# hiroharu-kato/neural_renderer

Hardware: AMD Instinct MI355X
Metric: rasterize fwd+bwd Mpixels/sec @256x256 batch=64 (higher is better)
Workload: dtype f32

## Files before the change

### include/nr_hip.h

```cpp
#ifndef NR_HIP_H
#define NR_HIP_H

#include <stddef.h>
#include <stdint.h>

#ifdef __cplusplus
extern "C" {
#endif

#define NR_VERSION 600

#define NR_E_NULL (-1)
#define NR_E_SIZE (-2)
#define NR_E_WORKSPACE (-3)
#define NR_E_MODE (-4)
#define NR_E_INDEX (-6)

#define NR_FLAG_FIX_TEXTURE_BATCH_Z 1
#define NR_FLAG_EXACT_GRADIENT 2
#define NR_FLAG_K6_GLOBAL 4
#define NR_FLAG_K6_SCAN 8

#define NR_FLAG_ZBUF_EPOCH 16
#define NR_ZBUF_EPOCH_FLAGS(e) (NR_FLAG_ZBUF_EPOCH | (((e) & 0xff) << 8))
#define NR_FLAG_SPARSE_WEIGHT_MAP 32
#define NR_FLAG_SERIAL_BACKWARD 64

#define NR_FLAG_K6_LEGACY 128
#define NR_FLAG_K6_PX 65536
#define NR_FLAG_SHARED_TEXTURES 131072


int nr_version(void);
const char *nr_error_string(int code);

size_t nr_forward_workspace_bytes(int32_t batch_size, int32_t num_faces, int32_t image_size);

size_t nr_backward_workspace_bytes(int32_t batch_size, int32_t num_faces, int32_t image_size,
                                   int32_t return_rgb, int32_t return_alpha);

int nr_forward_face_index_map(const float *faces, int32_t *face_index_map, float *weight_map, float *depth_map,
                              float *face_inv_map, uint8_t *visible_faces, int32_t batch_size, int32_t num_faces,
                              int32_t image_size, double near, double far, void *workspace, size_t workspace_bytes,
                              void *stream);

int nr_forward_texture_sampling(const float *faces, const float *faces_z_ref, const float *textures,
                                const int32_t *face_index_map, const float *weight_map, const float *depth_map,
                                float *rgb_map, int32_t *sampling_index_map, float *sampling_weight_map,
                                const float *background, int32_t bg_per_batch, float *alpha_map, int32_t batch_size,
                                int32_t num_faces, int32_t image_size, int32_t texture_size, double eps, int32_t flags,
                                void *stream);

int nr_backward_pixel_map(const float *faces, const int32_t *face_index_map, const float *rgb_map,
                          const float *alpha_map, const float *grad_rgb_map, const float *grad_alpha_map,
                          float *grad_faces, int32_t batch_size, int32_t num_faces, int32_t image_size, double eps,
                          int32_t return_rgb, int32_t return_alpha, int32_t flags, const uint8_t *visible_faces,
                          void *workspace, size_t workspace_bytes, void *stream);

int nr_backward_textures(const int32_t *face_index_map, const float *sampling_weight_map,
                         const int32_t *sampling_index_map, const float *faces, const float *faces_z_ref,
                         const float *weight_map, const float *depth_map, const float *grad_rgb_map, float *grad_textures,
                         int32_t batch_size, int32_t num_faces, int32_t image_size, int32_t texture_size, double eps,
// ... 473 lines not shown
```

### neural_renderer_amd/_lib.py

```python
import ctypes
import os

import torch

from . import _build

_CONTIGUOUS = torch.contiguous_format

_c = ctypes
_vp, _i32, _f64, _sz = _c.c_void_p, _c.c_int32, _c.c_double, _c.c_size_t


class Camera(_c.Structure):
    _fields_ = [('mode', _i32), ('perspective', _i32), ('target', _c.c_float * 3), ('up', _c.c_float * 3),
                ('width', _c.c_float)]


class Light(_c.Structure):
    _fields_ = [('intensity_ambient', _c.c_float), ('intensity_directional', _c.c_float),
                ('color_ambient', _c.c_float * 3), ('color_directional', _c.c_float * 3), ('direction', _c.c_float * 3)]


class FaceLight(_c.Structure):
    _fields_ = [('light', _vp), ('texture_faces', _i32), ('textures', _vp), ('grad_light', _vp)]
# ... 12 lines not shown
    _fields_ = [('images', _vp), ('image_table', _vp), ('faces_uv', _vp), ('face_image', _vp), ('base', _vp),
                ('texture_size', _i32), ('num_images', _i32), ('num_pixels', _i32), ('image_batch', _i32)]


class Lights(_c.Structure):
    _fields_ = [('intensity_ambient', _vp), ('intensity_directional', _vp), ('color_ambient', _vp),
                ('color_directional', _vp), ('direction', _vp), ('sh', _vp), ('per_image', _i32)]


class LightsGrad(_c.Structure):
    _fields_ = [('intensity_ambient', _vp), ('intensity_directional', _vp), ('color_ambient', _vp),
                ('color_directional', _vp), ('direction', _vp), ('sh', _vp)]


_cam_p, _light_p, _fl_p, _proj_p = _c.POINTER(Camera), _c.POINTER(Light), _c.POINTER(FaceLight), _c.POINTER(Projection)
_uv_p, _cl_p = _c.POINTER(UVImagesStruct), _c.POINTER(CornerLight)
_lights_p, _lights_grad_p = _c.POINTER(Lights), _c.POINTER(LightsGrad)

SIGNATURES = {
    'nr_version': (_c.c_int, []),
    'nr_error_string': (_c.c_char_p, [_c.c_int]),
    'nr_forward_workspace_bytes': (_sz, [_i32, _i32, _i32]),
    'nr_backward_workspace_bytes': (_sz, [_i32, _i32, _i32, _i32, _i32]),
    'nr_forward_face_index_map': (_c.c_int, [_vp] * 6 + [_i32, _i32, _i32, _f64, _f64, _vp, _sz, _vp]),
    'nr_forward_texture_sampling': (_c.c_int, [_vp] * 10 + [_i32, _vp, _i32, _i32, _i32, _i32, _f64, _i32, _vp]),
    'nr_backward_pixel_map': (_c.c_int, [_vp] * 7 + [_i32, _i32, _i32, _f64, _i32, _i32, _i32, _vp, _vp, _sz, _vp]),
    'nr_backward_textures': (_c.c_int, [_vp] * 9 + [_i32, _i32, _i32, _i32, _f64, _i32, _vp]),
    'nr_backward_depth_map': (_c.c_int, [_vp, _vp, _vp, _vp, _vp, _vp, _vp, _i32, _i32, _i32, _vp]),
    'nr_forward_rasterize': (_c.c_int, [_vp] * 10 + [_i32] * 5 + [_f64] * 3 + [_i32, _vp, _sz, _vp]),
    'nr_vertices_to_faces': (_c.c_int, [_vp, _vp, _vp, _i32, _i32, _i32, _i32, _vp]),
    'nr_vertices_to_faces_backward': (_c.c_int, [_vp, _vp, _vp, _i32, _i32, _i32, _i32, _vp]),
    'nr_backward_rasterize': (_c.c_int, [_vp] * 12 + [_i32] * 4 + [_f64, _i32, _vp, _vp, _sz, _vp]),
    'nr_image_epilogue': (_c.c_int, [_vp] * 6 + [_i32] * 3 + [_vp]),
    'nr_image_epilogue_backward': (_c.c_int, [_vp] * 6 + [_i32] * 3 + [_vp]),
    'nr_load_textures': (_c.c_int, [_vp] * 4 + [_i32] * 4 + [_vp]),
    'nr_create_texture_image': (_c.c_int, [_vp] * 3 + [_i32] * 5 + [_vp]),
    'nr_bake_uv_textures': (_c.c_int, [_vp] * 6 + [_i32] * 5 + [_vp]),
    'nr_uv_texture_map_workspace_bytes': (_sz, [_i32] * 4),
    'nr_uv_texture_map': (_c.c_int, [_vp] * 6 + [_i32] * 4 + [_vp, _sz, _vp]),
    'nr_bake_uv_textures_backward': (_c.c_int, [_vp] * 5 + [_i32] * 4 + [_vp]),
    'nr_forward_rasterize_uv': (_c.c_int, [_fl_p, _uv_p] + [_vp] * 8 + [_i32] * 4 + [_f64] * 3 + [_i32, _vp, _sz, _vp]),
    'nr_backward_uv_images_workspace_bytes': (_sz, [_i32] * 4),
    'nr_backward_uv_images': (_c.c_int, [_fl_p, _uv_p] + [_vp] * 6 + [_i32] * 3 + [_f64, _vp, _sz, _vp]),
    'nr_forward_rasterize_uv_smooth': (_c.c_int, [_cl_p, _uv_p] + [_vp] * 8 + [_i32] * 4 + [_f64] * 3 + [_i32, _vp, _sz, _vp]),
    'nr_backward_uv_images_smooth_workspace_bytes': (_sz, [_i32] * 4),
    'nr_backward_uv_images_smooth': (_c.c_int, [_cl_p, _uv_p] + [_vp] * 6 + [_i32] * 3 + [_f64, _vp, _sz, _vp]),
# ... 209 lines not shown
```

### neural_renderer_amd/csrc/nr_backward.hip

```cpp
#include "nr_device.h"
#include "nr_band_lines.h"
#include "nr_k6_tune.h"

using namespace nr;

int nr::plan_backward(const BackwardCall &c, BackwardPlan &p)
{
    p = {};
    const bool fused = c.stages == STAGE_ALL;
    const bool k6 = (c.stages & STAGE_K6) && (c.rgb || c.alpha);
    const bool k7 = (c.stages & STAGE_K7) && (!fused || (c.grad_rgb_map && c.grad_textures));
    const bool k8 = (c.stages & STAGE_K8) && (!fused || c.grad_depth_map);
    const bool sampled = c.sampling_weight_map != nullptr;
    if (!c.faces || !c.face_index_map) return NR_E_NULL;
    if ((c.stages & (STAGE_K6 | STAGE_K8)) && !c.grad_faces) return NR_E_NULL;
    if (c.stages == STAGE_K6 && !k6) return NR_E_MODE;
    if (k6 && c.rgb && (!c.rgb_map || !c.grad_rgb_map)) return NR_E_NULL;
    if (k6 && c.alpha && (!c.alpha_map || !c.grad_alpha_map)) return NR_E_NULL;
    if (k7) {
        if (!c.grad_rgb_map || !c.grad_textures) return NR_E_NULL;
        if ((c.sampling_index_map != nullptr) != sampled) return NR_E_MODE;
        if (!sampled && (!c.weight_map || !c.depth_map)) return NR_E_NULL;
    }
    if (k8 && (!c.depth_map || !c.weight_map || !c.grad_depth_map)) return NR_E_NULL;
    if (int e = check_sizes(c.B, c.F, c.S)) return e;
    if (k6 && (size_t)c.B * c.S * c.S > 0x7fffffffull / 3) return NR_E_SIZE;
    if (k7 && (c.ts < 2 || c.ts > 1024)) return NR_E_SIZE;
    if (k7 && c.lit.light && sampled) return NR_E_MODE;
    if (k7 && (c.flags & NR_FLAG_SHARED_TEXTURES)) return NR_E_MODE;

    const int B = c.B, F = c.F, ts = c.ts;
    p.k6 = k6;
    if (k6) {
        p.k6p = plan_k6(B, F, c.S, c.rgb, c.eps, c.flags);
        p.bands = p.k6p.kernel != K6_KERNEL_GLOBAL;
        if (p.bands && (!c.workspace || c.workspace_bytes < nr_backward_workspace_bytes(B, F, c.S, 1, 0))) return NR_E_WORKSPACE;
    }
    const bool fold = p.bands && k7 && ts <= 13;
    p.gather_first = fold && (size_t)B * F <= k6::SHARED_LAUNCH_MAX_FACES && !(c.flags & NR_FLAG_SERIAL_BACKWARD);
    const bool ts2_static = ts == 2 && (float)(1.0 - c.eps) < 1.0f;
    p.gather_in_tail = k6::TAIL_GATHER_MAX_FACES > 0 && fold && !p.gather_first && !(c.flags & NR_FLAG_SERIAL_BACKWARD) &&
                       ts2_static && !sampled && !c.lit.light && p.k6p.kernel == K6_KERNEL_ROW && !(c.flags & NR_FLAG_EXACT_GRADIENT) &&
                       !p.k6p.row_chunked && c.S <= 512 && (size_t)B * F <= k6::TAIL_GATHER_MAX_FACES;
    const bool gather_early = p.gather_first || p.gather_in_tail;
    p.face_zeros = gather_early ? FACE_ZEROS_ALL : (fold ? FACE_ZEROS_UNLISTED : FACE_ZEROS_NONE);
    p.finish = !p.bands ? FINISH_NONE : gather_early ? (ts <= 8 ? FINISH_BIG : FINISH_ADD) : (fold ? FINISH_GATHER : FINISH_KERNEL);

    if (k7) {
        const size_t n_tex = (size_t)ts * ts * ts * 3;
        p.static_taps = ts2_static && !sampled;
        p.gather = ts <= 13 ? GATHER_FACE : GATHER_ATOMIC;
        p.listed = p.bands && ts <= 13;
        p.lanes = p.static_taps ? 16 : (ts <= 5 ? 16 : (ts <= 8 ? 64 : 256));
        p.gather_lds = p.static_taps ? 0 : (size_t)(256 / p.lanes) * n_tex * sizeof(double);
        p.big = ts <= 8;
        p.depth_in_gather = k8 && ts <= 8 && !sampled && !(ts == 2 && !ts2_static);
        p.tex_bytes = (size_t)B * (c.lit.light ? c.lit.tex_faces : F) * n_tex * sizeof(float);
        if (p.gather_first) {
            p.setup_in_gather = p.k6p.use_records && k6_line_setup_args(c, p.k6p).lds_bytes <= 32768 && p.gather_lds <= 40960;
            if (p.setup_in_gather && !c.lit.light && ((size_t)c.grad_textures & 15) == 0) p.tex_zeros = TEX_ZEROS_SETUP;
        } else if (fold && p.tex_bytes % 16 == 0 && ((size_t)c.grad_textures & 15) == 0 && p.tex_bytes <= p.k6p.fill_max) {
            p.tex_zeros = p.gather_in_tail ? TEX_ZEROS_BAND_UNLISTED : TEX_ZEROS_BAND;
        }
        if (p.tex_zeros == TEX_ZEROS_NONE && (c.lit.light || p.listed || ts > 13)) p.tex_zeros = TEX_ZEROS_FILL;
        p.light_fill = c.lit.light && c.lit.grad_light;
    }
// ... 184 lines not shown
```

### neural_renderer_amd/csrc/nr_backward_pixel_map.hip

```cpp
#include "nr_device.h"
#include "nr_band_lines.h"
#include "nr_face_gather.h"
#include "nr_k6_tune.h"

#include <atomic>
#include <mutex>
#include <type_traits>

using namespace nr;

namespace {

enum { K6_FAST = 0, K6_EXACT_POW2 = 1, K6_EXACT = 2 };
#include "nr_k6_global.h"
#include "nr_k6_lists.h"
#include "nr_k6_fast.h"
#include "nr_k6_row.h"

__global__ __launch_bounds__(256) void k_bpm_finalize(const double *__restrict__ scratch, const int *__restrict__ slot_of,
                                                      float *__restrict__ grad_faces, int F, int n_faces_total, int add)
{
    const int i = blockIdx.x * blockDim.x + threadIdx.x;
    if (i >= n_faces_total) return;
    const int pos = slot_of[i];
// ... 68 lines not shown
        const int n_vis = f.vis_count[b];
        for (int slot = tid; slot < n_vis; slot += 256) {
            const size_t gi = (size_t)b * F + f.vis_list[(size_t)b * F + slot];
            const double *sc = f.scratch + ((size_t)b * F + slot) * 6;
            const float *fv = f.faces + gi * 9;
            const bool big = face_candidates(fv[0], fv[1], fv[3], fv[4], fv[6], fv[7], f.S).n > BIG_PX;
            float *gf = g.grad_faces + gi * 9;
#pragma unroll
            for (int v = 0; v < 3; v++) {
#pragma unroll
                for (int k = 0; k < 2; k++) {
                    const float k6v = (float)__hip_atomic_load(sc + 2 * v + k, __ATOMIC_RELAXED, __HIP_MEMORY_SCOPE_AGENT);
                    if (big) atomicAdd(gf + 3 * v + k, k6v);
                    else gf[3 * v + k] = k6v + gf[3 * v + k];
                }
            }
        }
    }
}


struct BpmLayout {
    size_t flags_off, scratch_off, count_off, chunk_off, cband_off, list_off, rng_off, slot_off, band_off, start_off, cursor_off, ok_off,
        ticket_off, lines_off, total, cap;
    int n_chunks;
};

size_t line_capacity(int F, int S)
{
    const size_t want = (size_t)8 * F + (size_t)32 * S + (size_t)(1.2 * (double)S * sqrt((double)F));
    return (want + 2047 - 1088) / 2048 * 2048 + 1088;
}

BpmLayout bpm_layout(int B, int F, int S)
{
    BpmLayout L;
    const size_t n = (size_t)B * F;
    L.flags_off = 0;
    L.scratch_off = align_up(n, 256);
    L.count_off = align_up(L.scratch_off + n * 6 * sizeof(double), 256);
    L.n_chunks = (F + VIS_CHUNK - 1) / VIS_CHUNK;
    L.chunk_off = L.count_off + align_up((size_t)B * sizeof(int), 256);
    L.cband_off = L.chunk_off + align_up((size_t)B * L.n_chunks * sizeof(int), 256);
    L.list_off = L.cband_off + (L.n_chunks <= SMALL_CHUNKS ? align_up((size_t)B * L.n_chunks * 2 * S * sizeof(int), 256) : 0);
    L.rng_off = L.list_off + align_up(n * sizeof(int), 256);
    L.slot_off = L.rng_off + align_up(n * 6 * sizeof(unsigned), 256);
    const size_t per_band = align_up((size_t)B * 2 * S * sizeof(int), 256);
    L.band_off = L.slot_off + align_up(n * sizeof(int), 256);
    L.start_off = L.band_off + per_band;
    L.cursor_off = L.start_off + per_band;
    L.ok_off = L.cursor_off + per_band;
    L.ticket_off = L.ok_off + align_up((size_t)B * sizeof(int), 256);
    L.lines_off = L.ticket_off + 256;
    L.cap = line_capacity(F, S);
    L.total = L.lines_off + (size_t)B * L.cap * sizeof(BandLine);
    return L;
}

struct ListsLayout {
    size_t count_off, list_off, total;
};
ListsLayout lists_layout(int B, int F)
{
    ListsLayout L;
    L.count_off = 0;
    L.list_off = align_up((size_t)B * sizeof(int), 256);
    L.total = L.list_off + (size_t)B * F * sizeof(int);
    return L;
}

BandShape band_shape(int S)
{
    if (S <= k6::SMALL_RASTER_MAX) return {256, 2, (size_t)40 * 1024};
    if (S > k6::WIDE_BUDGET_FROM && S <= k6::WIDE_BUDGET_TO) return {512, k6::WMAX, (size_t)80 * 1024};
    return {512, k6::WMAX, k6::LDS_BUDGET};
}
// ... 114 lines not shown
    const int B = c.B, F = c.F, S = c.S;
    const int CH = row_chunk(S, F), W = p.W_row;
    const unsigned n_ch = (unsigned)((S + CH - 1) / CH), total_wg = (unsigned)((S + W - 1) / W) * 2u * (unsigned)B * n_ch;
    auto go = [&](auto chunked) {
        return launch_lds<k_bpm_row<RGB, ALPHA, MODE, decltype(chunked)::value>>(
            dim3(xcd_grid(total_wg)), dim3(rowk::NT), p.row_lds, c.st, c.face_index_map, c.rgb_map, c.alpha_map, c.grad_rgb_map,
            c.grad_alpha_map, l.scratch, ls.band_lines, ls.band_start, ls.lines_ok, ls.line_buf, ls.cap, F, S, W, CH, (float)c.eps, c.eps, B,
            (uint4 *)zero_ptr, zero_bytes / 16);
    };
    return n_ch > 1 ? go(std::true_type()) : go(std::false_type());
}

template <bool RGB, bool ALPHA>
int launch_band_gather(const K6Plan &p, const BackwardCall &c, const BackwardPlan &bp, const K6Lists &l, const LineSetupArgs &ls,
                       void *fill, size_t fill_bytes)
{
    const int B = c.B, F = c.F, S = c.S, W = p.W_row;
    const unsigned total_wg = (unsigned)((S + W - 1) / W) * 2u * (unsigned)B, band_grid = xcd_grid(total_wg);
    const unsigned gather_x = ((unsigned)((F + 15) / 16) + k6::SLOT_STRIDE - 1) / k6::SLOT_STRIDE;
    BandRowArgs ra = {};
    ra.fi_map = c.face_index_map;   ra.rgb_map = c.rgb_map;         ra.alpha_map = c.alpha_map;
    ra.g_rgb = c.grad_rgb_map;      ra.g_alpha = c.grad_alpha_map;  ra.scratch = l.scratch;
    ra.band_lines = ls.band_lines;  ra.band_start = ls.band_start;  ra.lines_ok = ls.lines_ok;
    ra.line_buf = ls.line_buf;      ra.cap = ls.cap;                ra.B = B;
    ra.F = F;                       ra.S = S;                       ra.W = W;
    ra.CH = S;
    ra.eps_f = (float)c.eps;        ra.eps_d = c.eps;
    ra.zero16 = (uint4 *)fill;      ra.n_zero16 = fill_bytes / 16;  ra.zero_slot = l.slot_of;       ra.zero_epf = 6u;
    const FaceGatherArgs ga = face_gather_args(c, bp, l);
    auto go = [&](auto depth) {
        return launch_lds<k_band_gather<RGB, ALPHA, decltype(depth)::value>>(dim3(band_grid + gather_x * (unsigned)B), dim3(rowk::NT),
                                                                             p.row_lds, c.st, ra, ga, band_grid, gather_x);
    };
    return bp.depth_in_gather ? go(std::true_type()) : go(std::false_type());
}

int k6_row_band(int B, int F, int S, bool rgb, double eps, int flags, size_t *row_lds)
{
    const bool exact = (flags & NR_FLAG_EXACT_GRADIENT) != 0;
    const bool possible = !(flags & (NR_FLAG_K6_SCAN | NR_FLAG_K6_LEGACY)) && B <= 65535 && (exact || (float)eps >= 1e-30f);
    return possible ? row_band_config(S, F, rgb, exact, B, row_lds) : 0;
}

}

K6Plan nr::plan_k6(int B, int F, int S, bool rgb, double eps, int flags)
// ... 2 lines not shown
    const bool exact = (flags & NR_FLAG_EXACT_GRADIENT) != 0;
    p.mode = !exact ? K6_FAST : ((S & (S - 1)) == 0 ? K6_EXACT_POW2 : K6_EXACT);
    p.shape = band_shape(S);
    int w_max = p.shape.w_max, win = BAND_WIN;
    while (w_max > 1 && (size_t)B * 2 * ((S + w_max - 1) / w_max) < 3072) w_max >>= 1;
    p.W_fast = fast_band_config(S, rgb, p.shape, w_max, &p.fast_lds, &win, &p.qcap);
    if (p.W_fast == 0 || (flags & NR_FLAG_K6_GLOBAL)) {
        p.kernel = K6_KERNEL_GLOBAL;
        return p;
    }
    p.win_lines = min(win, max(4, min(BAND_WIN, (int)(65535ll * FSEG / (2ll * S))) & ~3));
    p.W_row = k6_row_band(B, F, S, rgb, eps, flags, &p.row_lds);
    const bool row = p.W_row > 0;
    p.kernel = row ? K6_KERNEL_ROW : K6_KERNEL_FAST;
    p.overflow_pass = row;
    p.row_chunked = row && row_chunk(S, F) < S;
    p.W = row ? 1 : p.W_fast;
    p.n_bands = (S + p.W - 1) / p.W;
    p.use_records = !(flags & NR_FLAG_K6_SCAN) && B <= 65535 && p.n_bands <= 3072;
    const int W_band = row ? p.W_row : p.W_fast;
    const size_t band_wgs = (size_t)((S + W_band - 1) / W_band) * 2 * (size_t)B;
    p.fill_max = band_wgs * ((size_t)k6::FOLD_KB << 10) * (size_t)(row ? rowk::NT : p.shape.threads) / 512;
    return p;
}

NR_API size_t nr_backward_workspace_bytes(int32_t B, int32_t F, int32_t S, int32_t return_rgb, int32_t return_alpha)
{
    if (check_sizes(B, F, S)) return 0;
    if (!return_rgb && !return_alpha) return lists_layout(B, F).total;
    return bpm_layout(B, F, S).total;
}

#ifdef NR_PROFILE_HOOK
#include "../../include/nr_hip_profile.h"
namespace {
struct BandKernelTimer {
    bool on = false, recorded = false;
    int which = -1;
    hipEvent_t start = nullptr, stop = nullptr;
} g_band_timer;
}

NR_API int nr_profile_band_kernel(int32_t enable)
{
    BandKernelTimer &t = g_band_timer;
    if (enable && !t.start) {
// ... 78 lines not shown
        const int lds_counters = n_bands <= 4096;
        hipLaunchKernelGGL(k_compact_visible, dim3((unsigned)L.n_chunks, (unsigned)B), dim3(VIS_CHUNK),
                           lds_counters ? (size_t)2 * n_bands * sizeof(int) : 0, st, vflags, chunk_count, vis_list, vis_count,
                           slot_of, F, L.n_chunks, c.faces, rng, scratch, S, band_lines, n_bands, W, lds_counters, zero_faces,
                           zero_listed);
        hipLaunchKernelGGL(k_band_scan, dim3((unsigned)B), dim3(256), 0, st, band_lines, band_start, band_cursor, lines_ok,
                           n_bands, plan.use_records ? L.cap : 0, 0, ticket);
    }
    return launch_status();
}

LineSetupArgs nr::k6_line_setup_args(const BackwardCall &c, const K6Plan &plan)
{
    const BpmLayout L = bpm_layout(c.B, c.F, c.S);
    unsigned char *ws = (unsigned char *)c.workspace;
    const int n_bands = plan.n_bands;
    const float k2s = (c.flags & NR_FLAG_EXACT_GRADIENT) ? 1.0f : 2.0f / (float)c.S;
    const unsigned slots = (unsigned)((c.F + LS_FACES - 1) / LS_FACES);
    const unsigned stride = (c.flags & NR_FLAG_SERIAL_BACKWARD) ? 1u : k6::SLOT_STRIDE;
    return {c.faces, c.face_index_map, (const int *)(ws + L.list_off), (const int *)(ws + L.count_off),
            (const unsigned *)(ws + L.rng_off), (const int *)(ws + L.cband_off), compact_in_one_launch(L, n_bands) ? L.n_chunks : 0,
            (int *)(ws + L.band_off), (int *)(ws + L.start_off), (int *)(ws + L.cursor_off), (int *)(ws + L.ok_off),
            (BandLine *)(ws + L.lines_off), L.cap, c.F, c.S, plan.W, n_bands, k2s, (slots + stride - 1) / stride,
            (unsigned)c.B, (size_t)6 * n_bands * sizeof(int)};
}

int nr::run_line_setup(const LineSetupArgs &a, hipStream_t st)
{
    const int rc = launch_lds<k_line_setup>(dim3(a.grid_x * a.grid_y), dim3(256), a.lds_bytes, st, a);
    return rc ? rc : launch_status();
}

int nr::k6_band(const BackwardCall &c, const K6Plan &plan, const K6Lists &l, const LineSetupArgs &ls, void *fill, size_t fill_bytes,
                const BackwardPlan *tail, bool overflow_later)
{
    if (plan.kernel == K6_KERNEL_GLOBAL)
        return with_k6_maps(c.rgb, c.alpha, [&](auto r, auto a) {
            hipLaunchKernelGGL((k_bpm_global<decltype(r)::value, decltype(a)::value>), dim3((unsigned)(c.B * c.F)), dim3(WAVE), 0,
                               c.st, c.faces, c.face_index_map, c.rgb_map, c.alpha_map, c.grad_rgb_map, c.grad_alpha_map,
                               c.grad_faces, c.F, c.S, c.eps);
            return launch_status();
        });
    auto band_fast = [&](auto overflow_only, void *zp, size_t zb) {
        return with_k6_types(c.rgb, c.alpha, plan.mode, [&](auto r, auto a, auto m) {
            return launch_fast<decltype(r)::value, decltype(a)::value, decltype(m)::value, decltype(overflow_only)::value>(
                plan, c, l, ls, zp, zb);
        });
// ... 65 lines not shown
```

### neural_renderer_amd/csrc/nr_band_lines.h

```cpp
#pragma once
#include "nr_device.h"

namespace nr {

struct __attribute__((aligned(16))) BandLine {
    int in_rng;
    int out_rng;
    int geo;
    int tgt;
    float cross, c0, c1;
    int fn;
};

struct LineSetupArgs {
    const float *faces;
    const int32_t *fi_map;
    const int *vis_list, *vis_count;
    const unsigned *rng;
    const int *chunk_band;
    int n_sum;
    int *band_lines, *band_start, *band_cursor, *lines_ok;
    BandLine *line_buf;
    size_t cap;
    int F, S, W, n_bands;
    float k2s;
    unsigned grid_x, grid_y;
    size_t lds_bytes;
};

namespace {


constexpr unsigned RNG_EMPTY = 1u;

__device__ __forceinline__ unsigned edge_range(float p0x, float p1x, int S)
{
    const int d0_from = (int)fmax((double)ceilf(fminf(p0x, p1x)), 0.0);
    const int d0_to = (int)fmin((double)fmaxf(p0x, p1x), S - 1.0);
    return (p0x != p1x && d0_to >= d0_from) ? (unsigned)d0_from | ((unsigned)d0_to << 16) : RNG_EMPTY;
}


struct LineHead {
    float p0x, p0y, p1x, p1y, p2x, p2y, d0f, d1_cross;
    int direction, d1_in, d1_out;
    bool live;
};

__device__ __forceinline__ void line_head_points(LineHead &h, const float *__restrict__ fv, int e, int axis, int d0, int S)
{
    const float fs = (float)S;
// ... 123 lines not shown
    int n_pos = bx < n_wg ? (n_vis - pos0 + pstep - 1) / pstep : 0;
    if (n_pos == 0 && !first) return;
    unsigned r_own = RNG_EMPTY;
    int fn_own = 0;
    if (tid < 6 * n_pos) {
        const int p = tid / 6, ae = tid - 6 * p, axis = ae / 3, e = ae - 3 * axis;
        r_own = rng[(((size_t)b * 2 + axis) * F + pos0 + p * pstep) * 3 + e];
    }
    if (tid < n_pos) fn_own = vis_list[(size_t)b * F + pos0 + tid * pstep];
    int ok;
    if (n_sum > 0) {
        const int total = band_sum_prefix(chunk_band + (size_t)b * n_sum * 2 * n_bands, n_sum, 2 * n_bands, s_cnt, s_start, s_tmp);
        ok = (size_t)total <= cap ? 1 : 0;
        if (first) {
            for (int i = tid; i < 2 * n_bands; i += 256) {
                band_lines[(size_t)b * 2 * n_bands + i] = s_cnt[i];
                band_start[(size_t)b * 2 * n_bands + i] = s_start[i];
            }
            if (tid == 0) lines_ok[b] = ok;
        }
    } else {
        ok = lines_ok[b];
        for (int i = tid; i < 2 * n_bands; i += 256) s_start[i] = band_start[(size_t)b * 2 * n_bands + i];
    }
    if (n_pos == 0 || !ok) return;
    const int tid_all = tid;
    for (;;) {
    int tid = tid_all;
    asm volatile("" : "+v"(tid));
    __syncthreads();
    for (int i = tid; i < 2 * n_bands; i += 256) s_cnt[i] = 0;
    if (tid < 6 * LS_FACES) s_rng[tid] = r_own;
    if (tid < LS_FACES) s_fn[tid] = fn_own;
    __syncthreads();
    float fv_a = 0.0f, fv_b = 0.0f;
    {
        const int p = tid / 9, k = tid - 9 * p;
        if (p < n_pos) fv_a = faces[((size_t)b * F + s_fn[p]) * 9 + k];
        const int t2 = tid + 256, p2 = t2 / 9, k2 = t2 - 9 * p2;
        if (t2 < 9 * LS_FACES && p2 < n_pos) fv_b = faces[((size_t)b * F + s_fn[p2]) * 9 + k2];
    }
    {
        int lines = 0;
        if (tid < 6 * n_pos) {
            const int p = tid / 6, ae = tid - 6 * p, axis = ae / 3;
            const unsigned pr = s_rng[tid];
// ... 93 lines not shown
```

### neural_renderer_amd/csrc/nr_device.h

```cpp
#pragma once
#include <hip/hip_runtime.h>
#include <stdint.h>
#include <stdlib.h>

#include "../../include/nr_hip.h"

#define NR_API extern "C" __attribute__((visibility("default")))

namespace nr {

constexpr int WAVE = 64;


__device__ __forceinline__ bool is_backside(float x0, float y0, float x1, float y1, float x2, float y2)
{
    return (y2 - y0) * (x1 - x0) < (y1 - y0) * (x2 - x0);
}

__device__ __forceinline__ float to_pixel(float v, float fs) { return 0.5f * (v * fs + fs - 1.0f); }

__device__ __forceinline__ void compute_face_inv(const float px[3], const float py[3], float inv[9])
{
    inv[0] = py[1] - py[2];
    inv[1] = px[2] - px[1];
// ... 374 lines not shown
    const unsigned char *visible_faces;
    void *workspace;
    size_t workspace_bytes;
    FaceLight lit;
    hipStream_t st;
};

struct BandShape {
    int threads;
    int w_max;
    size_t budget;
};
enum K6Kernel { K6_KERNEL_FAST = 0, K6_KERNEL_ROW = 1, K6_KERNEL_GLOBAL = 2 };
struct K6Plan {
    int kernel;
    int mode;
    BandShape shape;
    int W_fast;
    size_t fast_lds;
    int win_lines, qcap;
    int W_row;
    size_t row_lds;
    int W, n_bands;
    bool use_records;
    bool overflow_pass;
    bool row_chunked;
    size_t fill_max;
};
K6Plan plan_k6(int B, int F, int S, bool rgb, double eps, int flags);

enum FaceZeros { FACE_ZEROS_NONE, FACE_ZEROS_UNLISTED, FACE_ZEROS_ALL };
enum TexZeros { TEX_ZEROS_NONE, TEX_ZEROS_BAND, TEX_ZEROS_SETUP, TEX_ZEROS_FILL, TEX_ZEROS_BAND_UNLISTED };
enum K6Finish { FINISH_NONE, FINISH_KERNEL, FINISH_GATHER, FINISH_BIG, FINISH_ADD };
enum Gather { GATHER_NONE, GATHER_FACE, GATHER_ATOMIC };

struct BackwardPlan {
    bool k6;
    K6Plan k6p;
    bool bands;
    int face_zeros;
    bool gather_first;
    bool gather_in_tail;
    bool setup_alone;
    bool setup_in_gather;
    int tex_zeros;
    size_t tex_bytes;
// ... 44 lines not shown
```

### neural_renderer_amd/csrc/nr_k6_row.h

```cpp

__device__ __forceinline__ int window_team(int n_rec, int n_parts, int nsl)
{
    const int n_win = (n_rec + 63) >> 6;
    if (nsl < 32) return 1;
    int team = n_parts;
    while (team > 1 && n_parts / team < n_win) team >>= 1;
    return team;
}

__device__ __forceinline__ void wave_lds_handover()
{
    __builtin_amdgcn_fence(__ATOMIC_RELEASE, "wavefront");
    __builtin_amdgcn_wave_barrier();
    __builtin_amdgcn_fence(__ATOMIC_ACQUIRE, "wavefront");
}

namespace rowk {
constexpr int NT = 256, NW = NT / 64;
constexpr int WIN = 64;
constexpr int SEG = 16;
constexpr int MAX_SEGS = 64;
constexpr int IN_SEG = 16;
constexpr int IN_BATCH = 4;
constexpr int MAX_PX = 1024;
// ... 7 lines not shown
}

#ifdef NR_ROW_STATS
__device__ unsigned long long g_row_stats[8];
NR_API int nr_dev_row_stats(unsigned long long *out8)
{
    if (hipMemcpyFromSymbol(out8, HIP_SYMBOL(g_row_stats), sizeof(unsigned long long) * 8) != hipSuccess) return 1;
    unsigned long long z[8] = {0, 0, 0, 0, 0, 0, 0, 0};
    return hipMemcpyToSymbol(HIP_SYMBOL(g_row_stats), z, sizeof(z)) == hipSuccess ? 0 : 1;
}
#define NR_ROW_STAT(i, v) do { if (lane == 0) atomicAdd(&g_row_stats[i], (unsigned long long)(v)); } while (0)
constexpr unsigned NR_ROW_DUMP_WINDOWS = 1u << 16;
__device__ unsigned g_row_dump_n;
__device__ unsigned g_row_dump[NR_ROW_DUMP_WINDOWS * 64];
NR_API int nr_dev_row_dump(unsigned *out, unsigned *n_windows)
{
    if (hipMemcpyFromSymbol(n_windows, HIP_SYMBOL(g_row_dump_n), sizeof(unsigned)) != hipSuccess) return 1;
    const unsigned n = *n_windows < NR_ROW_DUMP_WINDOWS ? *n_windows : NR_ROW_DUMP_WINDOWS, zero = 0;
    if (n && hipMemcpyFromSymbol(out, HIP_SYMBOL(g_row_dump), (size_t)n * 64 * sizeof(unsigned)) != hipSuccess) return 1;
    return hipMemcpyToSymbol(HIP_SYMBOL(g_row_dump_n), &zero, sizeof(unsigned)) == hipSuccess ? 0 : 1;
}
#else
#define NR_ROW_STAT(i, v) ((void)0)
#endif

struct BandRowArgs {
    const int32_t *fi_map;
    const float *rgb_map, *alpha_map, *g_rgb, *g_alpha;
    double *scratch;
    const int *band_lines, *band_start, *lines_ok;
    const BandLine *line_buf;
    size_t cap;
    int F, S, W, B;
    float eps_f;
    double eps_d;
    uint4 *zero16;
    size_t n_zero16;
    const int *zero_slot;
    unsigned zero_epf;
    int CH;
};

template <bool RGB, bool ALPHA, int MODE, bool CHUNKED, bool UNLISTED>
__device__ __forceinline__ void bpm_row_body(
    const int32_t *__restrict__ fi_map, const float *__restrict__ rgb_map, const float *__restrict__ alpha_map,
    const float *__restrict__ g_rgb, const float *__restrict__ g_alpha, double *__restrict__ scratch,
    const int *__restrict__ band_lines, const int *__restrict__ band_start, const int *__restrict__ lines_ok,
    const BandLine *__restrict__ line_buf, size_t cap, int F, int S, int W, int CH, float eps_f, double eps_d, int B,
    uint4 *__restrict__ zero16, size_t n_zero16, const int *__restrict__ zero_slot, unsigned zero_epf)
{
    using namespace rowk;
    constexpr bool EXACT = MODE != K6_FAST;
    extern __shared__ __attribute__((aligned(16))) unsigned char smem[];
    const int tid = threadIdx.x, lane = tid & 63, wave = rfl(tid >> 6);
    const unsigned n_bands = (unsigned)(S + W - 1) / (unsigned)W, n_ch = CHUNKED ? (unsigned)(S + CH - 1) / (unsigned)CH : 1u;
    const unsigned total_wg = n_bands * 2u * (unsigned)B * n_ch;
    const unsigned logical = xcd_block(total_wg);
    if (logical >= total_wg) return;
    if (n_zero16) {
        const size_t per = (n_zero16 + total_wg - 1) / total_wg, z_lo = (size_t)logical * per, z_hi = min(n_zero16, z_lo + per);
        for (size_t k = z_lo + tid; k < z_hi; k += NT) {
            if constexpr (UNLISTED) { if (zero_slot[k / zero_epf] >= 0) continue; }
            zero16[k] = make_uint4(0u, 0u, 0u, 0u);
        }
    }
    const unsigned bandidx = logical / n_ch;
    const int c0 = CHUNKED ? (int)(logical - bandidx * n_ch) * CH : 0, SL = CHUNKED ? min(CH, S - c0) : S;
    const int band = (int)(bandidx % n_bands), axis = (int)((bandidx / n_bands) & 1u);
    int b = (int)(bandidx / (2u * n_bands));
    if constexpr (UNLISTED && k6::ROW_DEAL_IMAGES) {
        const int q = B >> 3;
        if ((B & 7) == 0 && q >= 2) b = (b % q) * 8 + b / q;
    }
    if (lines_ok[b] == 0) return;
    const int band_lo = band * W, nld = min(W, S - band_lo);
    const size_t lt = ((size_t)b * 2 + axis) * S + band_lo;
    int n_tot = 0;
    for (int l = 0; l < nld; ++l) n_tot += band_lines[lt + l];
    if (n_tot == 0) return;

    constexpr int NC = RGB ? 4 : 1;
    const int SP = (SL + 31) & ~31, nsl = SP / SEG;
    const unsigned npx = (unsigned)(W * SP), G_BYTES = (unsigned)g_bytes<RGB>(npx), C_BYTES = (unsigned)c_bytes<RGB, EXACT>(npx), FI_BYTES = npx * 4u;
    float *const s_g = (float *)smem;
    float *const s_p = (float *)(smem + G_BYTES);
    int *const s_fi = (int *)(smem + G_BYTES + C_BYTES);
    float4 *const s_k = (float4 *)(smem + G_BYTES + C_BYTES + FI_BYTES);
    unsigned char *wave_mem = smem + G_BYTES + C_BYTES + FI_BYTES + (EXACT ? 0u : (unsigned)K_BYTES) + (unsigned)wave * WAVE_BYTES;
    double2 *acc = (double2 *)wave_mem;
    int *hist = (int *)wave_mem;
    const int n_parts = max(1, NW / W);
    const BandLine *recs_b = line_buf + (size_t)b * cap;
    const size_t img = (size_t)b * S * S;
    auto map_index = [&](int ld, int d1) { return axis ? img + (size_t)(band_lo + ld) * S + (c0 + d1) : img + (size_t)(c0 + d1) * S + band_lo + ld; };
    auto map_colour = [&](size_t gi) {
        float4 c = make_float4(0.0f, 0.0f, 0.0f, 0.0f);
        if constexpr (!RGB || ALPHA) c.x = alpha_map[gi];
        if constexpr (RGB) { c.y = rgb_map[3 * gi]; c.z = rgb_map[3 * gi + 1]; c.w = rgb_map[3 * gi + 2]; }
        return c;
    };
    auto line_k = [&](int ld) {
        if constexpr (EXACT) return make_float4(0.0f, 0.0f, 0.0f, 0.0f);
// ... 451 lines not shown
                const bool neg0 = EXACT || (((__float_as_uint(qq.y) >> 31) != 0) != tneg);
                const bool neg1 = EXACT || (((__float_as_uint(qq.z) >> 31) != 0) != tneg);
                const double t0 = (flags & 2) ? in0 + (neg0 ? a.x : -a.x) : 0.0;
                const double t1 = (flags & 4) ? in1 + (neg1 ? a.y : -a.y) : 0.0;
                const int tgt = hh.w, lpos = tgt & 0x0fffffff;
                double *dst = scratch + ((size_t)b * F + lpos) * 6 + (1 - axis);
                if (t0 != 0.0) atomicAdd(dst + 2 * ((tgt >> 28) & 3), t0);
                if (t1 != 0.0) atomicAdd(dst + 2 * ((tgt >> 30) & 3), t1);
            }
            wave_lds_handover();
        }
    }
}

template <bool RGB, bool ALPHA, int MODE, bool CHUNKED>
__global__ __launch_bounds__(rowk::NT, MODE == K6_FAST ? 5 : 4) void k_bpm_row(
    const int32_t *__restrict__ fi_map, const float *__restrict__ rgb_map, const float *__restrict__ alpha_map,
    const float *__restrict__ g_rgb, const float *__restrict__ g_alpha, double *__restrict__ scratch,
    const int *__restrict__ band_lines, const int *__restrict__ band_start, const int *__restrict__ lines_ok,
    const BandLine *__restrict__ line_buf, size_t cap, int F, int S, int W, int CH, float eps_f, double eps_d, int B,
    uint4 *__restrict__ zero16, size_t n_zero16)
{
    bpm_row_body<RGB, ALPHA, MODE, CHUNKED, false>(fi_map, rgb_map, alpha_map, g_rgb, g_alpha, scratch, band_lines, band_start, lines_ok,
                                                   line_buf, cap, F, S, W, CH, eps_f, eps_d, B, zero16, n_zero16, nullptr, 1u);
}

template <bool RGB, bool ALPHA, bool DEPTH>
__global__ __launch_bounds__(rowk::NT, 5) void k_band_gather(BandRowArgs r, FaceGatherArgs g, unsigned band_grid, unsigned gather_x)
{
    if (blockIdx.x < band_grid) {
        bpm_row_body<RGB, ALPHA, K6_FAST, false, true>(r.fi_map, r.rgb_map, r.alpha_map, r.g_rgb, r.g_alpha, r.scratch, r.band_lines,
                                                       r.band_start, r.lines_ok, r.line_buf, r.cap, r.F, r.S, r.W, r.CH, r.eps_f, r.eps_d,
                                                       r.B, r.zero16, r.n_zero16, r.zero_slot, r.zero_epf);
    } else {
        const SlotImage w = image_fastest(blockIdx.x - band_grid, (unsigned)r.B);
        const int n_vis = g.vis_count[w.by];
        for (int bx = w.bx; bx * 16 < n_vis; bx += (int)gather_x) face_gather_body<true, DEPTH, false>(g, bx, w.by);
    }
}
```

### neural_renderer_amd/csrc/nr_k6_tune.h

```cpp
#pragma once

#ifndef NR_K6_FB
#define NR_K6_FB 3
#endif
#ifndef NR_K6_U_GROUP
#define NR_K6_U_GROUP 3
#endif
#ifndef NR_K6_SMALL_RASTER_MAX
#define NR_K6_SMALL_RASTER_MAX 400
#endif
#ifndef NR_K6_MINWAVES_256
#define NR_K6_MINWAVES_256 4
#endif
#ifndef NR_K6_WMAX
#define NR_K6_WMAX 4
#endif
#ifndef NR_K6_FOLD_KB
#define NR_K6_FOLD_KB 128
#endif
#ifndef NR_K6_LDS_BUDGET
#define NR_K6_LDS_BUDGET (53 * 1024)
#endif

#ifndef NR_K6_WIDE_BUDGET_FROM
// ... 10 lines not shown
#endif
#ifndef NR_ROW_MIN_WGS_1
#define NR_ROW_MIN_WGS_1 1024
#endif

#ifndef NR_SHARED_LAUNCH_MAX_FACES
#define NR_SHARED_LAUNCH_MAX_FACES 98304
#endif
#ifndef NR_TAIL_GATHER_MAX_FACES
#define NR_TAIL_GATHER_MAX_FACES 655360
#endif
#ifndef NR_SLOT_STRIDE
#define NR_SLOT_STRIDE 4
#endif
#ifndef NR_MERGE_OVERFLOW
#define NR_MERGE_OVERFLOW 1
#endif
#ifndef NR_SETUP_GATHER_IMAGE_FASTEST
#define NR_SETUP_GATHER_IMAGE_FASTEST 1
#endif
#ifndef NR_ROW_DEAL_IMAGES
#define NR_ROW_DEAL_IMAGES 1
#endif

namespace nr {
namespace k6 {
constexpr bool ROW_DEAL_IMAGES = NR_ROW_DEAL_IMAGES != 0;
constexpr unsigned SLOT_STRIDE = NR_SLOT_STRIDE;
static_assert(SLOT_STRIDE >= 1, "slots per workgroup of the strided launches");
constexpr bool MERGE_OVERFLOW = NR_MERGE_OVERFLOW != 0;
constexpr int FB = NR_K6_FB;
constexpr int U_GROUP = NR_K6_U_GROUP;
static_assert(U_GROUP >= 1 && U_GROUP <= 4, "a super-piece's count travels in two bits");
constexpr int SMALL_RASTER_MAX = NR_K6_SMALL_RASTER_MAX;
constexpr int MINWAVES_256 = NR_K6_MINWAVES_256;
constexpr int WMAX = NR_K6_WMAX;
constexpr int FOLD_KB = NR_K6_FOLD_KB;
constexpr unsigned long LDS_BUDGET = NR_K6_LDS_BUDGET;
constexpr unsigned long ROW_MIN_WGS = NR_ROW_MIN_WGS, ROW_MIN_WGS_1 = NR_ROW_MIN_WGS_1;
constexpr unsigned OVF_GRID = NR_K6_OVF_GRID;
constexpr int WIDE_BUDGET_FROM = NR_K6_WIDE_BUDGET_FROM, WIDE_BUDGET_TO = NR_K6_WIDE_BUDGET_TO;
constexpr unsigned long SHARED_LAUNCH_MAX_FACES = NR_SHARED_LAUNCH_MAX_FACES;
constexpr unsigned long TAIL_GATHER_MAX_FACES = NR_TAIL_GATHER_MAX_FACES;
}
}
```

Measured before the change: 16610.

## Precompute per-image band order words for the row backward and skip empty bands

Line setup now writes, per image, an order table of band words that pack the band's axis, index and total line count. The fused band/gather kernel reads that word instead of summing band_lines per workgroup, and exits early for empty bands. With the default ROW_BAND_ORDER=0 the order is the identity. Optional modes sort bands by load (rank by total) so heavy bands are scheduled first. An optional timeline instrumentation path is also added. The change costs extra workspace and a setup pass over band counts.

```diff
diff --git a/include/nr_hip.h b/include/nr_hip.h
--- a/include/nr_hip.h
+++ b/include/nr_hip.h
@@ -38,6 +38,8 @@
 
 size_t nr_backward_workspace_bytes(int32_t batch_size, int32_t num_faces, int32_t image_size,
                                    int32_t return_rgb, int32_t return_alpha);
+
+size_t nr_backward_band_order_offset(int32_t batch_size, int32_t num_faces, int32_t image_size);
 
 int nr_forward_face_index_map(const float *faces, int32_t *face_index_map, float *weight_map, float *depth_map,
                               float *face_inv_map, uint8_t *visible_faces, int32_t batch_size, int32_t num_faces,
diff --git a/neural_renderer_amd/_lib.py b/neural_renderer_amd/_lib.py
--- a/neural_renderer_amd/_lib.py
+++ b/neural_renderer_amd/_lib.py
@@ -58,6 +58,7 @@
     'nr_error_string': (_c.c_char_p, [_c.c_int]),
     'nr_forward_workspace_bytes': (_sz, [_i32, _i32, _i32]),
     'nr_backward_workspace_bytes': (_sz, [_i32, _i32, _i32, _i32, _i32]),
+    'nr_backward_band_order_offset': (_sz, [_i32, _i32, _i32]),
     'nr_forward_face_index_map': (_c.c_int, [_vp] * 6 + [_i32, _i32, _i32, _f64, _f64, _vp, _sz, _vp]),
     'nr_forward_texture_sampling': (_c.c_int, [_vp] * 10 + [_i32, _vp, _i32, _i32, _i32, _i32, _f64, _i32, _vp]),
     'nr_backward_pixel_map': (_c.c_int, [_vp] * 7 + [_i32, _i32, _i32, _f64, _i32, _i32, _i32, _vp, _vp, _sz, _vp]),
diff --git a/neural_renderer_amd/csrc/nr_backward.hip b/neural_renderer_amd/csrc/nr_backward.hip
--- a/neural_renderer_amd/csrc/nr_backward.hip
+++ b/neural_renderer_amd/csrc/nr_backward.hip
@@ -42,6 +42,7 @@
     p.gather_in_tail = k6::TAIL_GATHER_MAX_FACES > 0 && fold && !p.gather_first && !(c.flags & NR_FLAG_SERIAL_BACKWARD) &&
                        ts2_static && !sampled && !c.lit.light && p.k6p.kernel == K6_KERNEL_ROW && !(c.flags & NR_FLAG_EXACT_GRADIENT) &&
                        !p.k6p.row_chunked && c.S <= 512 && (size_t)B * F <= k6::TAIL_GATHER_MAX_FACES;
+    p.k6p.W_order = p.gather_in_tail ? p.k6p.W_row : 0;
     const bool gather_early = p.gather_first || p.gather_in_tail;
     p.face_zeros = gather_early ? FACE_ZEROS_ALL : (fold ? FACE_ZEROS_UNLISTED : FACE_ZEROS_NONE);
     p.finish = !p.bands ? FINISH_NONE : gather_early ? (ts <= 8 ? FINISH_BIG : FINISH_ADD) : (fold ? FINISH_GATHER : FINISH_KERNEL);
diff --git a/neural_renderer_amd/csrc/nr_backward_pixel_map.hip b/neural_renderer_amd/csrc/nr_backward_pixel_map.hip
--- a/neural_renderer_amd/csrc/nr_backward_pixel_map.hip
+++ b/neural_renderer_amd/csrc/nr_backward_pixel_map.hip
@@ -114,7 +114,7 @@
 
 struct BpmLayout {
     size_t flags_off, scratch_off, count_off, chunk_off, cband_off, list_off, rng_off, slot_off, band_off, start_off, cursor_off, ok_off,
-        ticket_off, lines_off, total, cap;
+        ticket_off, order_off, lines_off, total, cap;
     int n_chunks;
 };
 
@@ -143,7 +143,8 @@
     L.cursor_off = L.start_off + per_band;
     L.ok_off = L.cursor_off + per_band;
     L.ticket_off = L.ok_off + align_up((size_t)B * sizeof(int), 256);
-    L.lines_off = L.ticket_off + 256;
+    L.order_off = L.ticket_off + 256;
+    L.lines_off = L.order_off + per_band;
     L.cap = line_capacity(F, S);
     L.total = L.lines_off + (size_t)B * L.cap * sizeof(BandLine);
     return L;
@@ -304,6 +305,8 @@
     ra.fi_map = c.face_index_map;   ra.rgb_map = c.rgb_map;         ra.alpha_map = c.alpha_map;
     ra.g_rgb = c.grad_rgb_map;      ra.g_alpha = c.grad_alpha_map;  ra.scratch = l.scratch;
     ra.band_lines = ls.band_lines;  ra.band_start = ls.band_start;  ra.lines_ok = ls.lines_ok;
+    if (!ls.band_order || ls.order_W != W) return NR_E_MODE;
+    ra.band_order = ls.band_order;
     ra.line_buf = ls.line_buf;      ra.cap = ls.cap;                ra.B = B;
     ra.F = F;                       ra.S = S;                       ra.W = W;
     ra.CH = S;
@@ -352,6 +355,12 @@
     const size_t band_wgs = (size_t)((S + W_band - 1) / W_band) * 2 * (size_t)B;
     p.fill_max = band_wgs * ((size_t)k6::FOLD_KB << 10) * (size_t)(row ? rowk::NT : p.shape.threads) / 512;
     return p;
+}
+
+NR_API size_t nr_backward_band_order_offset(int32_t B, int32_t F, int32_t S)
+{
+    if (check_sizes(B, F, S)) return 0;
+    return bpm_layout(B, F, S).order_off;
 }
 
 NR_API size_t nr_backward_workspace_bytes(int32_t B, int32_t F, int32_t S, int32_t return_rgb, int32_t return_alpha)
@@ -476,7 +485,8 @@
             (const unsigned *)(ws + L.rng_off), (const int *)(ws + L.cband_off), compact_in_one_launch(L, n_bands) ? L.n_chunks : 0,
             (int *)(ws + L.band_off), (int *)(ws + L.start_off), (int *)(ws + L.cursor_off), (int *)(ws + L.ok_off),
             (BandLine *)(ws + L.lines_off), L.cap, c.F, c.S, plan.W, n_bands, k2s, (slots + stride - 1) / stride,
-            (unsigned)c.B, (size_t)6 * n_bands * sizeof(int)};
+            (unsigned)c.B, (size_t)6 * n_bands * sizeof(int),
+            plan.W_order > 0 ? (unsigned *)(ws + L.order_off) : nullptr, plan.W_order};
 }
 
 int nr::run_line_setup(const LineSetupArgs &a, hipStream_t st)
diff --git a/neural_renderer_amd/csrc/nr_band_lines.h b/neural_renderer_amd/csrc/nr_band_lines.h
--- a/neural_renderer_amd/csrc/nr_band_lines.h
+++ b/neural_renderer_amd/csrc/nr_band_lines.h
@@ -1,5 +1,6 @@
 #pragma once
 #include "nr_device.h"
+#include "nr_k6_tune.h"
 
 namespace nr {
 
@@ -26,7 +27,16 @@
     float k2s;
     unsigned grid_x, grid_y;
     size_t lds_bytes;
+    unsigned *band_order;
+    int order_W;
 };
+
+constexpr unsigned ORDER_AXIS_SHIFT = 10, ORDER_TOTAL_SHIFT = 11, ORDER_TOTAL_MAX = (1u << 21) - 1u;
+__host__ __device__ constexpr unsigned band_order_word(int axis, int band, int total)
+{
+    return (unsigned)band | ((unsigned)axis << ORDER_AXIS_SHIFT) |
+           (((unsigned)total < ORDER_TOTAL_MAX ? (unsigned)total : ORDER_TOTAL_MAX) << ORDER_TOTAL_SHIFT);
+}
 
 namespace {
 
@@ -196,6 +206,33 @@
     } else {
         ok = lines_ok[b];
         for (int i = tid; i < 2 * n_bands; i += 256) s_start[i] = band_start[(size_t)b * 2 * n_bands + i];
+        if (first && a.order_W > 0) {
+            for (int i = tid; i < 2 * n_bands; i += 256) s_cnt[i] = band_lines[(size_t)b * 2 * n_bands + i];
+            __syncthreads();
+        }
+    }
+    if (first && a.order_W > 0) {
+        const int Wo = a.order_W, nbo = (S + Wo - 1) / Wo, n2o = 2 * nbo;
+        for (int i = tid; i < n2o; i += 256) {
+            const int axis = i / nbo, lo = (i - axis * nbo) * Wo, hi = min(S, lo + Wo);
+            int t = 0;
+            for (int l = lo; l < hi; ++l) t += s_cnt[axis * n_bands + l];
+            s_base[i] = ok ? t : 0;
+        }
+        __syncthreads();
+        for (int i = tid; i < n2o; i += 256) {
+            const int t = s_base[i], axis = i / nbo;
+            int rank = 0;
+            if constexpr (k6::ROW_BAND_ORDER <= 0) {
+                rank = i;
+            } else {
+                for (int k = 0; k < n2o; ++k) {
+                    const int tk = s_base[k];
+                    rank += (tk > t || (tk == t && k < i)) ? 1 : 0;
+                }
+            }
+            a.band_order[(size_t)b * n2o + rank] = band_order_word(axis, i - axis * nbo, t);
+        }
     }
     if (n_pos == 0 || !ok) return;
     const int tid_all = tid;
diff --git a/neural_renderer_amd/csrc/nr_device.h b/neural_renderer_amd/csrc/nr_device.h
--- a/neural_renderer_amd/csrc/nr_device.h
+++ b/neural_renderer_amd/csrc/nr_device.h
@@ -420,6 +420,7 @@
     int W_row;
     size_t row_lds;
     int W, n_bands;
+    int W_order;
     bool use_records;
     bool overflow_pass;
     bool row_chunked;
diff --git a/neural_renderer_amd/csrc/nr_k6_row.h b/neural_renderer_amd/csrc/nr_k6_row.h
--- a/neural_renderer_amd/csrc/nr_k6_row.h
+++ b/neural_renderer_amd/csrc/nr_k6_row.h
@@ -53,6 +53,27 @@
 }
 #else
 #define NR_ROW_STAT(i, v) ((void)0)
+#endif
+
+#ifdef NR_ROW_TIMELINE
+constexpr unsigned NR_ROW_TL_MAX = 1u << 16;
+__device__ unsigned long long g_row_tl[NR_ROW_TL_MAX * 4];
+NR_API int nr_dev_row_timeline(unsigned long long *out, unsigned n_workgroups)
+{
+    const unsigned n = n_workgroups < NR_ROW_TL_MAX ? n_workgroups : NR_ROW_TL_MAX;
+    return hipMemcpyFromSymbol(out, HIP_SYMBOL(g_row_tl), (size_t)n * 4 * sizeof(unsigned long long)) == hipSuccess ? 0 : 1;
+}
+__device__ __forceinline__ void row_tl_id(unsigned logical, bool gather, int b, int axis, int band, unsigned n_rec)
+{
+    if (threadIdx.x != 0 || blockIdx.x >= NR_ROW_TL_MAX) return;
+    g_row_tl[4 * (size_t)blockIdx.x + 2] = (unsigned long long)logical | ((unsigned long long)(blockIdx.x % NUM_XCD) << 32) |
+                                            ((unsigned long long)(gather ? 1 : 0) << 63);
+    g_row_tl[4 * (size_t)blockIdx.x + 3] = (unsigned long long)(unsigned)b | ((unsigned long long)(unsigned)axis << 16) |
+                                            ((unsigned long long)(unsigned)band << 17) | ((unsigned long long)n_rec << 32);
+}
+#define NR_ROW_TL_ID(logical, gather, b, axis, band, n_rec) row_tl_id(logical, gather, b, axis, band, n_rec)
+#else
+#define NR_ROW_TL_ID(logical, gather, b, axis, band, n_rec) ((void)0)
 #endif
 
 struct BandRowArgs {
@@ -70,6 +91,7 @@
     const int *zero_slot;
     unsigned zero_epf;
     int CH;
+    const unsigned *band_order;
 };
 
 template <bool RGB, bool ALPHA, int MODE, bool CHUNKED, bool UNLISTED>
@@ -78,7 +100,8 @@
     const float *__restrict__ g_rgb, const float *__restrict__ g_alpha, double *__restrict__ scratch,
     const int *__restrict__ band_lines, const int *__restrict__ band_start, const int *__restrict__ lines_ok,
     const BandLine *__restrict__ line_buf, size_t cap, int F, int S, int W, int CH, float eps_f, double eps_d, int B,
-    uint4 *__restrict__ zero16, size_t n_zero16, const int *__restrict__ zero_slot, unsigned zero_epf)
+    uint4 *__restrict__ zero16, size_t n_zero16, const int *__restrict__ zero_slot, unsigned zero_epf,
+    const unsigned *__restrict__ band_order)
 {
     using namespace rowk;
     constexpr bool EXACT = MODE != K6_FAST;
@@ -97,18 +120,39 @@
     }
     const unsigned bandidx = logical / n_ch;
     const int c0 = CHUNKED ? (int)(logical - bandidx * n_ch) * CH : 0, SL = CHUNKED ? min(CH, S - c0) : S;
-    const int band = (int)(bandidx % n_bands), axis = (int)((bandidx / n_bands) & 1u);
+    int band = (int)(bandidx % n_bands), axis = (int)((bandidx / n_bands) & 1u);
     int b = (int)(bandidx / (2u * n_bands));
-    if constexpr (UNLISTED && k6::ROW_DEAL_IMAGES) {
+    constexpr bool ORDERED = UNLISTED && !CHUNKED && k6::ROW_BAND_ORDER >= 0;
+    if constexpr (ORDERED) {
+        unsigned rank = bandidx % (2u * n_bands);
         const int q = B >> 3;
-        if ((B & 7) == 0 && q >= 2) b = (b % q) * 8 + b / q;
-    }
-    if (lines_ok[b] == 0) return;
+        if (k6::ROW_BAND_ORDER == 2 && (B & 7) == 0) {
+            const unsigned x = (unsigned)(b / q), l = bandidx - x * (unsigned)q * 2u * n_bands;
+            rank = l / (unsigned)q;
+            b = (int)(x * (unsigned)q + (l - rank * (unsigned)q));
+        }
+        if (k6::ROW_DEAL_IMAGES && (B & 7) == 0 && q >= 2) b = (b % q) * 8 + b / q;
+        const unsigned word = band_order[(size_t)b * 2u * n_bands + rank];
+        band = (int)(word & ((1u << ORDER_AXIS_SHIFT) - 1u));
+        axis = (int)((word >> ORDER_AXIS_SHIFT) & 1u);
+        NR_ROW_TL_ID(logical, false, b, axis, band, word >> ORDER_TOTAL_SHIFT);
+        if ((word >> ORDER_TOTAL_SHIFT) == 0u) return;
+    } else {
+        if constexpr (UNLISTED && k6::ROW_DEAL_IMAGES) {
+            const int q = B >> 3;
+            if ((B & 7) == 0 && q >= 2) b = (b % q) * 8 + b / q;
+        }
+        NR_ROW_TL_ID(logical, false, b, axis, band, 0u);
+        if (lines_ok[b] == 0) return;
+    }
     const int band_lo = band * W, nld = min(W, S - band_lo);
     const size_t lt = ((size_t)b * 2 + axis) * S + band_lo;
-    int n_tot = 0;
-    for (int l = 0; l < nld; ++l) n_tot += band_lines[lt + l];
-    if (n_tot == 0) return;
+    if constexpr (!ORDERED) {
+        int n_tot = 0;
+        for (int l = 0; l < nld; ++l) n_tot += band_lines[lt + l];
+        if (n_tot == 0) return;
+        NR_ROW_TL_ID(logical, false, b, axis, band, (unsigned)n_tot);
+    }
 
     constexpr int NC = RGB ? 4 : 1;
     const int SP = (SL + 31) & ~31, nsl = SP / SEG;
@@ -606,19 +650,30 @@
     uint4 *__restrict__ zero16, size_t n_zero16)
 {
     bpm_row_body<RGB, ALPHA, MODE, CHUNKED, false>(fi_map, rgb_map, alpha_map, g_rgb, g_alpha, scratch, band_lines, band_start, lines_ok,
-                                                   line_buf, cap, F, S, W, CH, eps_f, eps_d, B, zero16, n_zero16, nullptr, 1u);
+                                                   line_buf, cap, F, S, W, CH, eps_f, eps_d, B, zero16, n_zero16, nullptr, 1u, nullptr);
 }
 
 template <bool RGB, bool ALPHA, bool DEPTH>
 __global__ __launch_bounds__(rowk::NT, 5) void k_band_gather(BandRowArgs r, FaceGatherArgs g, unsigned band_grid, unsigned gather_x)
 {
+#ifdef NR_ROW_TIMELINE
+    const unsigned long long tl_entry = wall_clock64();
+#endif
     if (blockIdx.x < band_grid) {
         bpm_row_body<RGB, ALPHA, K6_FAST, false, true>(r.fi_map, r.rgb_map, r.alpha_map, r.g_rgb, r.g_alpha, r.scratch, r.band_lines,
                                                        r.band_start, r.lines_ok, r.line_buf, r.cap, r.F, r.S, r.W, r.CH, r.eps_f, r.eps_d,
-                                                       r.B, r.zero16, r.n_zero16, r.zero_slot, r.zero_epf);
+                                                       r.B, r.zero16, r.n_zero16, r.zero_slot, r.zero_epf, r.band_order);
     } else {
         const SlotImage w = image_fastest(blockIdx.x - band_grid, (unsigned)r.B);
         const int n_vis = g.vis_count[w.by];
+        NR_ROW_TL_ID(blockIdx.x - band_grid, true, w.by, 0, w.bx, w.bx * 16 < n_vis ? 1u : 0u);
         for (int bx = w.bx; bx * 16 < n_vis; bx += (int)gather_x) face_gather_body<true, DEPTH, false>(g, bx, w.by);
     }
-}
+#ifdef NR_ROW_TIMELINE
+    __syncthreads();
+    if (threadIdx.x == 0 && blockIdx.x < NR_ROW_TL_MAX) {
+        g_row_tl[4 * (size_t)blockIdx.x] = tl_entry;
+        g_row_tl[4 * (size_t)blockIdx.x + 1] = wall_clock64();
+    }
+#endif
+}
diff --git a/neural_renderer_amd/csrc/nr_k6_tune.h b/neural_renderer_amd/csrc/nr_k6_tune.h
--- a/neural_renderer_amd/csrc/nr_k6_tune.h
+++ b/neural_renderer_amd/csrc/nr_k6_tune.h
@@ -56,9 +56,14 @@
 #ifndef NR_ROW_DEAL_IMAGES
 #define NR_ROW_DEAL_IMAGES 1
 #endif
+#ifndef NR_ROW_BAND_ORDER
+#define NR_ROW_BAND_ORDER 0
+#endif
 
 namespace nr {
 namespace k6 {
+constexpr int ROW_BAND_ORDER = NR_ROW_BAND_ORDER;
+static_assert(ROW_BAND_ORDER >= -1 && ROW_BAND_ORDER <= 2, "the band orders of bpm_row_body");
 constexpr bool ROW_DEAL_IMAGES = NR_ROW_DEAL_IMAGES != 0;
 constexpr unsigned SLOT_STRIDE = NR_SLOT_STRIDE;
 static_assert(SLOT_STRIDE >= 1, "slots per workgroup of the strided launches");
```

Result: no change. 16750, median of 6 (+0.9%).
